# omricarmi/FastHEVC

Measured on AMD Instinct MI355X. Metric: CTU depth decisions/sec at 1080p all-intra + BD-rate delta vs full-RDO HM, higher is better.
Workload: dtype int8 operands / int32 accumulate on v_mfma_i32_32x32x32_i8 (conv2, conv3: 93 % of the MACs); conv1 bf16 operands / f32 accumulate (fixed-point valued); every result exact

## Files before the change

### fasthevc_amd/csrc/k_cnn.hip

```cpp
#include "fhevc_internal.h"
#include <algorithm>
#include <cstdlib>
#include <cstring>

typedef __attribute__((ext_vector_type(8))) short bf16x8;
typedef __attribute__((ext_vector_type(8))) _Float16 f16x8;
typedef __attribute__((ext_vector_type(16))) float f32x16;
typedef __attribute__((ext_vector_type(2))) unsigned short u16x2;

namespace {

constexpr int A1_ROW = 36 * 16;
constexpr int A1_EVEN = 19 * 16;
constexpr int R1_OFF = 0;
constexpr int A3_OFF = R1_OFF;
constexpr int A2_PITCH = 18;
constexpr int A2_PLANE = 18 * 18 * 16 + 192;
constexpr int IN_PITCH = 68;
#ifndef FHEVC_I8_PRIO
#define FHEVC_I8_PRIO 0x0222
#endif
#ifndef FHEVC_F16_PRIO
#define FHEVC_F16_PRIO 0x0123
#endif
// ... 2 lines not shown
#define FHEVC_PRIO_ON(phase)  if (FHEVC_PRIO_OF(phase)) { if (I8) FHEVC_SETPRIO_DYN(1 + prio_slot) else __builtin_amdgcn_s_setprio(FHEVC_PRIO_OF(phase)); }
#define FHEVC_PRIO_OFF(phase) if (FHEVC_PRIO_OF(phase)) __builtin_amdgcn_s_setprio(0);
#ifndef FHEVC_I8_C2_FILL_POOL
#define FHEVC_I8_C2_FILL_POOL 0
#endif
#ifndef FHEVC_I8_C2_FILL_REQUANT
#define FHEVC_I8_C2_FILL_REQUANT 0
#endif
#ifndef FHEVC_I8_C3_FILL
#define FHEVC_I8_C3_FILL 4
#endif
#ifndef FHEVC_I8_C2_FENCE
#define FHEVC_I8_C2_FENCE 0
#endif
#ifndef FHEVC_F16_C2_FILL_POOL
#define FHEVC_F16_C2_FILL_POOL 1
#endif
#ifndef FHEVC_F16_C2_FILL_REQUANT
#define FHEVC_F16_C2_FILL_REQUANT 3
#endif
#ifndef FHEVC_F16_C2_FENCE
#define FHEVC_F16_C2_FENCE 1
#endif
#ifndef FHEVC_I8_C2_SCHED
#define FHEVC_I8_C2_SCHED 1
#endif
#ifndef FHEVC_I8_C3_SCHED
#define FHEVC_I8_C3_SCHED 0
#endif
#ifndef FHEVC_F16_C3_SCHED
#define FHEVC_F16_C3_SCHED 1
#endif
#ifndef FHEVC_CONV1_UNROLL
#define FHEVC_CONV1_UNROLL 2
#endif
#ifndef FHEVC_I8_WG_PER_CU
#define FHEVC_I8_WG_PER_CU 3
#endif
template <bool I8>
struct Lds {
  static constexpr int A1_PLANE = (I8 ? 35 : 34) * A1_ROW;
  static constexpr int A1_PLANES = I8 ? 1 : 2, A2_PLANES = I8 ? 2 : 4;
  static constexpr int R1_BYTES = A1_PLANES * A1_PLANE;
  static constexpr int R2_OFF = R1_OFF + R1_BYTES;
  static constexpr int R2_BYTES = A2_PLANES * A2_PLANE;
  static constexpr int BIAS_OFF = R2_OFF + R2_BYTES;
  static constexpr int LOGIT_OFF = BIAS_OFF + 112 * 4;
  static constexpr int HEADW_OFF = LOGIT_OFF + 64 * 4;
  static constexpr int HADP_OFF = HEADW_OFF + 18432;
  static constexpr int HEADX_OFF = HADP_OFF + 1024;
  static constexpr int LDS_BYTES = HEADX_OFF + 768;
  static constexpr unsigned HALO_FILL = I8 ? 0x80808080u : 0u;
  static_assert(A2_PLANE % 256 == 0, "conv3 reads lane groups of a ds_read_b128 from different planes");
  static_assert(33 * IN_PITCH * 4 + 4 * IN_PITCH * 4 <= R2_BYTES, "input tile (and conv1's one fragment read past it) must fit the A2 region");
  static_assert(HEADW_OFF % 16 == 0, "head weights are read with ds_read_b128");
  static_assert(A3_OFF + 16384 <= R1_OFF + R1_BYTES, "conv3's output must fit R1");
  static_assert(R2_OFF + R2_BYTES <= 65536, "halo offsets are packed into 16 bits");
};
static_assert(2 * Lds<false>::LDS_BYTES <= 160 * 1024, "two workgroups per CU");
static_assert(3 * Lds<true>::LDS_BYTES <= 160 * 1024, "three workgroups per CU");
constexpr int A1_PLANE = Lds<false>::A1_PLANE;

constexpr int HEAD64_OFF = 0, HEAD32_OFF = 2 * 4096, HEAD16_OFF = 4 * 4096;
constexpr int HEADM_OFF = 2 * 4096, HEADM_STEP = 10 * 64, HEADM_BYTES = 16 * HEADM_STEP;

__device__ __forceinline__ float max_with_xor1(float v)
{
  const int o = __builtin_amdgcn_update_dpp(0, __builtin_bit_cast(int, v), 0xB1, 0xF, 0xF, true);
// ... 547 lines not shown
  const int pl = e / 68, k0 = e - pl * 68;
  int y, x;
  if (k0 < 18) { y = 0; x = k0; }
  else if (k0 < 36) { y = 17; x = k0 - 18; }
  else { const int k = k0 - 36; y = 1 + (k >> 1); x = (k & 1) ? 17 : 0; }
  return Lds<I8>::R2_OFF + pl * A2_PLANE + (y * A2_PITCH + x) * 16;
}
template <bool I8>
__device__ __forceinline__ int in_halo_off(int e)
{
  int y, x;
  if (e < 66) { y = 0; x = e; }
  else if (e < 132) { y = 65; x = e - 66; }
  else { const int k = e - 132; y = 1 + (k >> 1); x = (k & 1) ? 65 : 0; }
  return Lds<I8>::R2_OFF + 2 * (2 * ((y >> 1) * IN_PITCH + x) + (y & 1));
}
struct HaloCells { unsigned a1, a2, in; };
template <bool I8>
__device__ __forceinline__ HaloCells halo_cells(int tid)
{
  constexpr int N1 = 132 * Lds<I8>::A1_PLANES, N2 = 68 * Lds<I8>::A2_PLANES;
  HaloCells hc;
  hc.a1 = (unsigned)a1_halo_off<I8>(min(tid, N1 - 1)) | ((unsigned)a1_halo_off<I8>(min(tid + 256, N1 - 1)) << 16);
  hc.a2 = (unsigned)a2_halo_off<I8>(min(tid, N2 - 1)) | ((unsigned)a2_halo_off<I8>(min(tid + 256, N2 - 1)) << 16);
  hc.in = (unsigned)in_halo_off<I8>(tid) | ((unsigned)in_halo_off<I8>(min(tid + 256, 259)) << 16);
  return hc;
}
template <bool I8>
__device__ __forceinline__ void zero_a1_halo(unsigned char* lds, int tid, unsigned cells)
{
  asm volatile("" : "+v"(cells));
  constexpr unsigned Z = Lds<I8>::HALO_FILL;
  *reinterpret_cast<uint4*>(lds + (cells & 0xFFFF)) = make_uint4(Z, Z, Z, Z);
  if (tid < 132 * Lds<I8>::A1_PLANES - 256) *reinterpret_cast<uint4*>(lds + (cells >> 16)) = make_uint4(Z, Z, Z, Z);
}

__device__ __forceinline__ unsigned long long stamp()
{
  unsigned long long t;
  __builtin_amdgcn_sched_barrier(0);
  asm volatile("s_memtime %0\n\ts_waitcnt lgkmcnt(0)" : "=s"(t)::"memory");
  __builtin_amdgcn_sched_barrier(0);
  return t;
}

#define FHEVC_PHASE_IDS                                   \
  int tid = (int)threadIdx.x;                             \
  asm volatile("" : "+v"(tid));                           \
  if (TRIO) tid &= 255;                                   \
  const int lane = tid & 63, wave = tid >> 6;             \
  const int r = lane & 31, h = lane >> 5;                 \
  (void)r; (void)h; (void)wave;

template <bool STAMPS, int HAD, int ARITH, int TRIO = 0>
__global__ __launch_bounds__(TRIO ? 768 : 256, TRIO ? 1 : (ARITH ? FHEVC_I8_WG_PER_CU : 2)) void fhevc_cnn_depth_kernel(FhevcFrames F, FhevcCnnWeights W,
                                                                  uint8_t* __restrict__ d_depth, int32_t* __restrict__ d_had,
                                                                  int32_t* __restrict__ d_logits,
                                                                  uint32_t* __restrict__ d_flags,
                                                                  unsigned long long* __restrict__ d_stamps,
                                                                  uint8_t* __restrict__ d_depth_max, int margin_split, int margin_stop)
{
  extern __shared__ __attribute__((aligned(16))) unsigned char lds_all[];
  const int group = TRIO ? __builtin_amdgcn_readfirstlane((int)(threadIdx.x >> 8)) : 0;
  unsigned char* const lds = lds_all + (TRIO ? group * Lds<ARITH != 0>::LDS_BYTES : 0);
  const int vgrid = TRIO ? 3 * (int)gridDim.x : (int)gridDim.x;
  const int vbidx = TRIO ? group * (int)gridDim.x + (int)blockIdx.x : (int)blockIdx.x;
  __builtin_amdgcn_s_setreg((1 << 11) | 1, 2);
  const int tid = TRIO ? (int)(threadIdx.x & 255) : (int)threadIdx.x;
  const int lane = tid & 63, wave = tid >> 6;
  constexpr bool I8 = ARITH != 0, FASTRQ = ARITH == 2;
  int prio_slot = 0;
  if (I8) {
    const unsigned la = __builtin_amdgcn_s_getreg((31 << 11) | 6);
    const unsigned base = la & 0xFFFu, sz = (la >> 12) & 0x1FFu;
    prio_slot = base >= 2 * sz && sz ? 2 : (base >= sz && sz ? 1 : 0);
    if (TRIO) prio_slot = group;
  }
  (void)prio_slot;
  constexpr bool MFMA_HEADS = I8;
  (void)FASTRQ;
  using L = Lds<I8>;
  const HaloCells hc = halo_cells<I8>(tid);
  const int hb64a = W.bhead[0], hb64b = W.bhead[1] + W.bhead[6 + 0 * 52 + F.qp];
  const int hb32a = W.bhead[2], hb32b = W.bhead[3] + W.bhead[6 + 1 * 52 + F.qp];
  const int hb16a = W.bhead[4], hb16b = W.bhead[5] + W.bhead[6 + 2 * 52 + F.qp];
  const uint4* frag1p = W.frag + FHEVC_FRAG_CONV1 + lane;
  bf16x8 wA1a = __builtin_bit_cast(bf16x8, frag1p[0]);
// ... 106 lines not shown
  if (vblock < total) {
    stage_ctu(lds, L::R2_OFF, pre, F, pos, tid, ld_row, ld_seg, shift_in, hc.in);
    zero_a1_halo<I8>(lds, tid, hc.a1);
    if (HAD == 1) {
      const int hs = F.sample_bytes == 2 ? wave_src_hadamard<2>(pre, lane) : wave_src_hadamard<1>(pre, lane);
      if (lane == 0) logitL[56 + wave] = hs;
    }
  }
  __syncthreads();
  FHEVC_STAMP(0)
  float4 early_b0, early_b1;
  bf16x8 early_bq;
#define FHEVC_CONV1_EARLY_READS                                                                          \
  {                                                                                                      \
    FHEVC_PHASE_IDS                                                                                      \
    early_b0 = *reinterpret_cast<const float4*>(biasL + 8 * h);                                          \
    early_b1 = *reinterpret_cast<const float4*>(biasL + 8 * h + 4);                                      \
    const unsigned char* p = lds + L::R2_OFF + (2 * r + 2 * h) * 4 + wave * (IN_PITCH * 4);              \
    const uint2 lo = *reinterpret_cast<const uint2*>(p);                                                 \
    const uint2 hi = *reinterpret_cast<const uint2*>(p + IN_PITCH * 4);                                  \
    early_bq = __builtin_bit_cast(bf16x8, make_uint4(lo.x, lo.y, hi.x, hi.y));                           \
  }
  FHEVC_CONV1_EARLY_READS
  bf16x8 wH[5];
#define FHEVC_HAD_FRAG_LOADS                                                                                                              \
  if (HAD == 2) {                                                                                                                         \
    unsigned hoff = (unsigned)(threadIdx.x & 63) * 16u + (unsigned)((threadIdx.x >> 6) & 1) * (5u * 64u * 16u);   \
    asm volatile("" : "+v"(hoff));                                                                                                        \
    const unsigned char* hf = reinterpret_cast<const unsigned char*>(W.frag + FHEVC_FRAG_HAD) + hoff;                                     \
    _Pragma("unroll") for (int st = 0; st < 5; ++st) wH[st] = __builtin_bit_cast(bf16x8, *reinterpret_cast<const uint4*>(hf + st * 64 * 16)); \
  }
  FHEVC_HAD_FRAG_LOADS

  if (TRIO) {
    for (int i = 0; i < group; ++i) __syncthreads();
  }
  const int trio_iters = TRIO ? (total + vgrid - 1) / vgrid : 0;
  for (int work = vblock, it = 0; TRIO ? it < trio_iters : work < total; work += vgrid, ++it) {
    if (TRIO && work >= total) {
      __syncthreads(); __syncthreads(); __syncthreads(); __syncthreads();
      continue;
    }
    const int f = pos.f, cy = F.row_begin + pos.ry, cx = pos.cx;
    const CtuPos next = advance(pos, step, band_rows, F.ctus_x);


    {
      FHEVC_PHASE_IDS
      FHEVC_PRIO_ON(0)
      const unsigned char* inb = lds + L::R2_OFF + (2 * r + 2 * h) * 4;
      f32x16 bias1;
      {
        const float4 b0 = early_b0, b1 = early_b1;
        bias1[0] = b0.x; bias1[1] = b0.y; bias1[2] = b0.z; bias1[3] = b0.w;
        bias1[4] = b1.x; bias1[5] = b1.y; bias1[6] = b1.z; bias1[7] = b1.w;
#pragma unroll
        for (int i = 0; i < 8; ++i) bias1[8 + i] = bias1[i];
      }
      auto frag1 = [](const unsigned char* p) {
        const uint2 lo = *reinterpret_cast<const uint2*>(p);
        const uint2 hi = *reinterpret_cast<const uint2*>(p + IN_PITCH * 4);
        return __builtin_bit_cast(bf16x8, make_uint4(lo.x, lo.y, hi.x, hi.y));
      };
      const unsigned char* fp = inb + wave * (IN_PITCH * 4);
      unsigned char* dp = lds + R1_OFF + (I8 ? 8 * h : h * A1_PLANE) + (wave + 1) * A1_ROW + (((r + 1) & 1) ? 0 : A1_EVEN) + ((r + 1) >> 1) * 16;
      bf16x8 bq = early_bq;
      if (HAD == 2) {
        const int mt = wave & 1, nt = wave >> 1;
        const unsigned* hb = reinterpret_cast<const unsigned*>(lds + L::R2_OFF) + (16 * nt + 4 * (r >> 3)) * IN_PITCH + 8 * (r & 7) + 1 + 4 * h;
        f32x16 hacc;
#pragma unroll
        for (int k = 0; k < 16; ++k) hacc[k] = 0.0f;
#pragma unroll
        for (int st = 0; st < 5; ++st) {
          const unsigned* q = hb + st * IN_PITCH;
          const bf16x8 smp = __builtin_bit_cast(bf16x8, make_uint4(q[0], q[1], q[2], q[3]));
          hacc = __builtin_amdgcn_mfma_f32_32x32x16_bf16(wH[st], smp, hacc, 0, 0, 0);
        }
        float t = 0.0f;
#pragma unroll
        for (int k = 0; k < 16; ++k) t += __builtin_fabsf(hacc[k]);
        const u32x2_t sw = __builtin_amdgcn_permlane32_swap(__float_as_uint(t), __float_as_uint(t), false, false);
        t = __uint_as_float(sw.x) + __uint_as_float(sw.y);
        if (h == 0) reinterpret_cast<float*>(lds + L::HADP_OFF)[128 * had_set + 64 * mt + 32 * nt + r] = t;
      }
#pragma unroll FHEVC_CONV1_UNROLL
      for (int i = 0; i < 8; ++i) {
        const f32x16 acc0 = __builtin_amdgcn_mfma_f32_32x32x16_bf16(wA1a, bq, bias1, 0, 0, 0);
        const f32x16 acc1 = __builtin_amdgcn_mfma_f32_32x32x16_bf16(wA1b, bq, bias1, 0, 0, 0);
        fp += 4 * IN_PITCH * 4;
        bq = frag1(fp);
        if (I8) conv1_store_i8(acc0, acc1, dp);
        else conv1_store(acc0, acc1, dp);
        dp += 4 * A1_ROW;
      }
      FHEVC_PRIO_OFF(0)
    }
    __syncthreads();
    FHEVC_STAMP(1)

    if constexpr (I8) {
      FHEVC_PHASE_IDS
      FHEVC_PRIO_ON(1)
      constexpr unsigned Z = L::HALO_FILL;
      unsigned a2cells = hc.a2;
      asm volatile("" : "+v"(a2cells));
      *reinterpret_cast<uint4*>(lds + (a2cells & 0xFFFF)) = make_uint4(Z, Z, Z, Z);
      if (tid < 40) logitL[2 + tid] = tid < 8 ? ((tid & 1) ? hb32b : hb32a) : ((tid & 1) ? hb16b : hb16a);
      const int q = r >> 2;
      const int pr = (q ^ (q >> 1) ^ (q >> 2)) & 1, pc = ((r >> 3) << 2) | (r & 3);
      const unsigned char* a1p = lds + R1_OFF + (2 * pr + h) * A1_ROW + pc * 16;
      unsigned char* a2dst = lds + L::R2_OFF + ((pr + 1) * A2_PITCH + pc + 1) * 16 + 4 * h;
      const int u0 = wave, u1 = wave + 4;
      const unsigned char* h00 = a1p + (4 * u0) * A1_ROW;
      const unsigned char* h10 = a1p + (4 * u1) * A1_ROW;
      const int* b2t = reinterpret_cast<const int*>(biasL) + 16;
      i32x16 t0, t1, a0, a1;
      bf16x8 ring[RINGI];
      const int c2l = conv2_lane_i8(h);
      conv2_half_i8<true, false, 0>(h00, h00 + A1_ROW, c2l, wA2, ring, b2t, h, t0, t1);
      if (FHEVC_I8_C2_SCHED) __builtin_amdgcn_sched_group_barrier(0x100, RINGI + 4, 0);
      if (FHEVC_I8_C2_SCHED) sched_chain12_i8<0>();
      conv2_half_i8<false, false, C2F % RINGI>(h00 + A1_ROW, h10, c2l, wA2, ring, b2t, h, a0, a1);
      pool_h_i8(t0, t1);
// ... 215 lines not shown
        s64b = sdot4(a.x, d1.x, s64b); s64b = sdot4(a.y, d1.y, s64b); s64b = sdot4(a.z, d1.z, s64b); s64b = sdot4(a.w, d1.w, s64b);
      }
      const int r16a = dpp_row_sum(s16a), r16b = dpp_row_sum(s16b);
      const int r32a = dpp_row_sum(s32a), r32b = dpp_row_sum(s32b);
      const int r64a = dpp_row_sum(s64a), r64b = dpp_row_sum(s64b);
      if ((lane & 15) == 0) {
        const int bi = ((q >> 1) * 2 + (blk >> 1)) * 4 + (q & 1) * 2 + (blk & 1);
        *reinterpret_cast<int2*>(logitL + (5 + bi) * 2) = make_int2(r16a + hb16a, r16b + hb16b);
      }
      const int q32a = __builtin_amdgcn_readlane(r32a, 0) + __builtin_amdgcn_readlane(r32a, 16) +
                       __builtin_amdgcn_readlane(r32a, 32) + __builtin_amdgcn_readlane(r32a, 48);
      const int q32b = __builtin_amdgcn_readlane(r32b, 0) + __builtin_amdgcn_readlane(r32b, 16) +
                       __builtin_amdgcn_readlane(r32b, 32) + __builtin_amdgcn_readlane(r32b, 48);
      const int q64a = __builtin_amdgcn_readlane(r64a, 0) + __builtin_amdgcn_readlane(r64a, 16) +
                       __builtin_amdgcn_readlane(r64a, 32) + __builtin_amdgcn_readlane(r64a, 48);
      const int q64b = __builtin_amdgcn_readlane(r64b, 0) + __builtin_amdgcn_readlane(r64b, 16) +
                       __builtin_amdgcn_readlane(r64b, 32) + __builtin_amdgcn_readlane(r64b, 48);
      if (lane == 0) {
        *reinterpret_cast<int2*>(logitL + (1 + q) * 2) = make_int2(q32a + hb32a, q32b + hb32b);
        *reinterpret_cast<int2*>(logitL + 44 + 2 * q) = make_int2(q64a, q64b);
      }
    }
    FHEVC_STAMP(6)
    if (work + vgrid < total) {
      FHEVC_PHASE_IDS
      stage_ctu(lds, L::R2_OFF, pre, F, next, tid, tid >> 2, tid & 3, shift_in, hc.in);
    }
    FHEVC_STAMP(7)
    __syncthreads();
    FHEVC_STAMP(4)
    FHEVC_CONV1_EARLY_READS
    FHEVC_HAD_FRAG_LOADS

    {
      FHEVC_PHASE_IDS
      const int vw = min(64, F.width - cx * 64), vh = min(64, F.height - cy * 64);
      const int ux = tid & 15, uy = tid >> 4;
      const int4 pa = *reinterpret_cast<const int4*>(logitL + 44), pb = *reinterpret_cast<const int4*>(logitL + 48);
      const int2 l64 = make_int2(hb64a + pa.x + pa.z + pb.x + pb.z, hb64b + pa.y + pa.w + pb.y + pb.w);
      const int2 l32 = *reinterpret_cast<const int2*>(logitL + 2 * (1 + (uy >> 3) * 2 + (ux >> 3)));
      const int2 l16 = *reinterpret_cast<const int2*>(logitL + 2 * (5 + (uy >> 2) * 4 + (ux >> 2)));
      const bool e64 = (vw < 64) || (vh < 64);
      bool inside = true, e32 = false, e16 = false;
      if (e64) {
        inside = (ux * 4 < vw) && (uy * 4 < vh);
        e32 = ((ux >> 3) * 32 + 32 > vw) || ((uy >> 3) * 32 + 32 > vh);
        e16 = ((ux >> 2) * 16 + 16 > vw) || ((uy >> 2) * 16 + 16 > vh);
      }
      const int d64 = l64.y - l64.x, d32 = l32.y - l32.x, d16 = l16.y - l16.x;
      const long long o = (long long)(f * band_rows + (cy - F.row_begin)) * F.ctus_x + cx;
      {
        const bool s64 = e64 || d64 > margin_split, s32 = e32 || d32 > margin_split, s16 = e16 || d16 > margin_split;
        const int d = (inside && s64) ? (s32 ? (s16 ? 3 : 2) : 1) : 0;
        d_depth[o * 256 + tid] = (uint8_t)d;
      }
      if (d_depth_max != nullptr) {
        const bool s64 = e64 || d64 > -margin_stop, s32 = e32 || d32 > -margin_stop, s16 = e16 || d16 > -margin_stop;
        const int d = (inside && s64) ? (s32 ? (s16 ? 3 : 2) : 1) : 0;
        d_depth_max[o * 256 + tid] = (uint8_t)d;
      }
      if (d_logits != nullptr && tid < 42) d_logits[o * 42 + tid] = tid == 0 ? l64.x : (tid == 1 ? l64.y : logitL[tid]);
      if (HAD == 1 && tid == 64) {
        const int4 hp = *reinterpret_cast<const int4*>(logitL + 56 + 4 * had_set);
        d_had[o] = hp.x + hp.y + hp.z + hp.w;
      }
      if (HAD == 2 && wave == 1) {
        const float* hp = reinterpret_cast<const float*>(lds + L::HADP_OFF) + 128 * had_set + lane;
        const int sb = (int)(hp[0] + hp[64]);
        int v = dpp_row_sum((sb + 2) >> 2);
        v = __builtin_amdgcn_readlane(v, 0) + __builtin_amdgcn_readlane(v, 16) + __builtin_amdgcn_readlane(v, 32) + __builtin_amdgcn_readlane(v, 48);
        if (lane == 0) d_had[o] = v;
      }
      if (d_flags != nullptr && wave == 0) {
        const int k = lane;
        const int bi = k - 5, qq = k < 5 ? k - 1 : (bi >> 3) * 2 + ((bi >> 1) & 1);
        const int qx = (qq & 1) * 32, qy = (qq >> 1) * 32, bxx = (bi & 3) * 16, byy = (bi >> 2) * 16;
        const int2 a64 = l64;
        const bool n64 = (vw < 64) || (vh < 64) || (a64.y - a64.x > margin_split);
        bool bit = n64;
        if (k >= 1 && k < 21) {
          const int2 a32 = *reinterpret_cast<const int2*>(logitL + 2 * (1 + qq));
          const bool n32 = n64 && (qx < vw) && (qy < vh) && ((qx + 32 > vw) || (qy + 32 > vh) || (a32.y - a32.x > margin_split));
          bit = n32;
          if (k >= 5) {
            const int2 a16 = *reinterpret_cast<const int2*>(logitL + 2 * k);
            bit = n32 && (bxx < vw) && (byy < vh) && ((bxx + 16 > vw) || (byy + 16 > vh) || (a16.y - a16.x > margin_split));
          }
        }
        const unsigned long long m = __ballot(bit && k < 21);
        if (lane == 0) d_flags[o] = (uint32_t)(m & 0x1FFFFFu);
      }
      zero_a1_halo<I8>(lds, tid, hc.a1);
    }
    FHEVC_STAMP(5)
    had_set ^= 1;
    pos = next;
  }
  if (TRIO) {
    for (int i = group; i < 2; ++i) __syncthreads();
  }
  if (STAMPS) {
    unsigned long long treal1;
    const unsigned long long tclk1 = stamp();
    asm volatile("s_memrealtime %0\n\ts_waitcnt lgkmcnt(0)" : "=s"(treal1)::"memory");
    if (tid == 0) {
      for (int k = 0; k < 8; ++k) d_stamps[vbidx * FHEVC_STAMP_SLOTS + k] = tsum[k];
      d_stamps[vbidx * FHEVC_STAMP_SLOTS + 8] = tclk1 - tclk0;
      d_stamps[vbidx * FHEVC_STAMP_SLOTS + 9] = treal1 - treal0;
      d_stamps[vbidx * FHEVC_STAMP_SLOTS + 10] = (unsigned long long)prio_slot;
    }
  }
#undef FHEVC_STAMP
#undef FHEVC_CONV1_EARLY_READS
#undef FHEVC_HAD_FRAG_LOADS
}

__device__ __forceinline__ void depth_map_of_ctu(const FhevcFrames& F, const int* logitL, const int* hads, int tid, int lane, int wave, int f, int cy, int cx,
                                                 int band_rows, int hb64a, int hb64b, int margin_split, int margin_stop, uint8_t* __restrict__ d_depth,
                                                 uint8_t* __restrict__ d_depth_max, int32_t* __restrict__ d_logits, uint32_t* __restrict__ d_flags,
                                                 int32_t* __restrict__ d_had, bool had)
{
  const int vw = min(64, F.width - cx * 64), vh = min(64, F.height - cy * 64);
  const int ux = tid & 15, uy = tid >> 4;
  const int4 pa = *reinterpret_cast<const int4*>(logitL + 44), pb = *reinterpret_cast<const int4*>(logitL + 48);
  const int2 l64 = make_int2(hb64a + pa.x + pa.z + pb.x + pb.z, hb64b + pa.y + pa.w + pb.y + pb.w);
  const int2 l32 = *reinterpret_cast<const int2*>(logitL + 2 * (1 + (uy >> 3) * 2 + (ux >> 3)));
  const int2 l16 = *reinterpret_cast<const int2*>(logitL + 2 * (5 + (uy >> 2) * 4 + (ux >> 2)));
  const bool e64 = (vw < 64) || (vh < 64);
  bool inside = true, e32 = false, e16 = false;
  if (e64) {
    inside = (ux * 4 < vw) && (uy * 4 < vh);
    e32 = ((ux >> 3) * 32 + 32 > vw) || ((uy >> 3) * 32 + 32 > vh);
    e16 = ((ux >> 2) * 16 + 16 > vw) || ((uy >> 2) * 16 + 16 > vh);
  }
  const int d64 = l64.y - l64.x, d32 = l32.y - l32.x, d16 = l16.y - l16.x;
  const long long o = (long long)(f * band_rows + (cy - F.row_begin)) * F.ctus_x + cx;
  {
    const bool s64 = e64 || d64 > margin_split, s32 = e32 || d32 > margin_split, s16 = e16 || d16 > margin_split;
    const int d = (inside && s64) ? (s32 ? (s16 ? 3 : 2) : 1) : 0;
    d_depth[o * 256 + tid] = (uint8_t)d;
  }
  if (d_depth_max != nullptr) {
    const bool s64 = e64 || d64 > -margin_stop, s32 = e32 || d32 > -margin_stop, s16 = e16 || d16 > -margin_stop;
    const int d = (inside && s64) ? (s32 ? (s16 ? 3 : 2) : 1) : 0;
    d_depth_max[o * 256 + tid] = (uint8_t)d;
  }
// ... 34 lines not shown
  const int tid = threadIdx.x, uy = tid & 15, sub = tid >> 4;
  for (long long c = (long long)blockIdx.x * 16 + sub; c < total; c += (long long)gridDim.x * 16) {
    const int rem = (int)(c % per_frame), cy = rem / F.ctus_x, cx = rem - cy * F.ctus_x;
    const int vw = min(64, F.width - cx * 64), vh = min(64, F.height - cy * 64);
    const uint32_t w = flags[c];
    uint32_t out[4] = { 0, 0, 0, 0 };
    if (uy * 4 < vh && (w & 1u)) {
#pragma unroll
      for (int j = 0; j < 4; ++j) {
        const int q = (uy >> 3) * 2 + (j >> 1), bi = (uy >> 2) * 4 + j;
        const uint32_t d = ((w >> (1 + q)) & 1u) ? (((w >> (5 + bi)) & 1u) ? 3u : 2u) : 1u;
        const int nvalid = min(4, max(0, (vw >> 2) - 4 * j));
        out[j] = (d * 0x01010101u) & (nvalid >= 4 ? 0xFFFFFFFFu : ((1u << (8 * nvalid)) - 1u));
      }
    }
    *reinterpret_cast<uint4*>(depth + c * 256 + uy * 16) = make_uint4(out[0], out[1], out[2], out[3]);
  }
}

}

hipError_t fhevc_launch_expand_flags(const FhevcFrames& fr, const uint32_t* d_flags, uint8_t* d_depth, hipStream_t stream)
{
  const long long total = (long long)fr.ctus_x * fr.ctus_y * fr.num_frames;
  if (total <= 0) return hipSuccess;
  const long long groups = (total + 15) / 16;
  const int grid = (int)(groups < 8192 ? groups : 8192);
  hipLaunchKernelGGL(fhevc_expand_flags_kernel, dim3(grid), dim3(256), 0, stream, fr, d_flags, d_depth);
  return hipGetLastError();
}

hipError_t fhevc_cnn_prepare_device()
{
  hipError_t e = hipFuncSetAttribute(reinterpret_cast<const void*>(&fhevc_cnn_depth_kernel<false, 0, 0>), hipFuncAttributeMaxDynamicSharedMemorySize, Lds<false>::LDS_BYTES);
  if (e == hipSuccess) e = hipFuncSetAttribute(reinterpret_cast<const void*>(&fhevc_cnn_depth_kernel<false, 1, 0>), hipFuncAttributeMaxDynamicSharedMemorySize, Lds<false>::LDS_BYTES);
  if (e == hipSuccess) e = hipFuncSetAttribute(reinterpret_cast<const void*>(&fhevc_cnn_depth_kernel<false, 2, 0>), hipFuncAttributeMaxDynamicSharedMemorySize, Lds<false>::LDS_BYTES);
  if (e == hipSuccess) e = hipFuncSetAttribute(reinterpret_cast<const void*>(&fhevc_cnn_family_kernel<32, 64, 128>), hipFuncAttributeMaxDynamicSharedMemorySize, LdsFam<32, 64, 128>::LDS_BYTES);
  if (e == hipSuccess) e = hipFuncSetAttribute(reinterpret_cast<const void*>(&fhevc_cnn_family_kernel<16, 32, 64>), hipFuncAttributeMaxDynamicSharedMemorySize, LdsFam<16, 32, 64>::LDS_BYTES);
#define FHEVC_LAYER_LDS(KCV) \
  if (e == hipSuccess) e = hipFuncSetAttribute(reinterpret_cast<const void*>(&fhevc_layer_conv_kernel<KCV, false, true>), hipFuncAttributeMaxDynamicSharedMemorySize, 80 * 1024); \
  if (e == hipSuccess) e = hipFuncSetAttribute(reinterpret_cast<const void*>(&fhevc_layer_conv_kernel<KCV, true, true>), hipFuncAttributeMaxDynamicSharedMemorySize, 80 * 1024);
  FHEVC_LAYER_LDS(1) FHEVC_LAYER_LDS(2) FHEVC_LAYER_LDS(3) FHEVC_LAYER_LDS(4)
#undef FHEVC_LAYER_LDS
#define FHEVC_LAYER_FUSE(KCV) \
  if (e == hipSuccess) e = hipFuncSetAttribute(reinterpret_cast<const void*>(&fhevc_layer_conv_kernel<KCV, false, true, true>), hipFuncAttributeMaxDynamicSharedMemorySize, 80 * 1024); \
  if (e == hipSuccess) e = hipFuncSetAttribute(reinterpret_cast<const void*>(&fhevc_layer_conv_kernel<KCV, true, true, true>), hipFuncAttributeMaxDynamicSharedMemorySize, 80 * 1024);
  FHEVC_LAYER_FUSE(1) FHEVC_LAYER_FUSE(2)
#undef FHEVC_LAYER_FUSE
  if (e == hipSuccess) e = hipFuncSetAttribute(reinterpret_cast<const void*>(&fhevc_cnn_d2_kernel<1, 2, 3, false>), hipFuncAttributeMaxDynamicSharedMemorySize, LdsD2<1, 2, 3>::LDS_BYTES);
  if (e == hipSuccess) e = hipFuncSetAttribute(reinterpret_cast<const void*>(&fhevc_cnn_d2_kernel<1, 2, 3, true>), hipFuncAttributeMaxDynamicSharedMemorySize, LdsD2<1, 2, 3>::LDS_BYTES);
  if (e == hipSuccess) e = hipFuncSetAttribute(reinterpret_cast<const void*>(&fhevc_cnn_depth_kernel<false, 0, 2, 1>), hipFuncAttributeMaxDynamicSharedMemorySize, 3 * Lds<true>::LDS_BYTES);
  if (e == hipSuccess) e = hipFuncSetAttribute(reinterpret_cast<const void*>(&fhevc_cnn_depth_kernel<false, 1, 2, 1>), hipFuncAttributeMaxDynamicSharedMemorySize, 3 * Lds<true>::LDS_BYTES);
  if (e == hipSuccess) e = hipFuncSetAttribute(reinterpret_cast<const void*>(&fhevc_cnn_depth_kernel<true, 1, 2, 1>), hipFuncAttributeMaxDynamicSharedMemorySize, 3 * Lds<true>::LDS_BYTES);
  return e;
}

bool fhevc_cnn_can_fuse_hadamard(const FhevcFrames& fr)
{
  const size_t sb = (size_t)fr.sample_bytes;
  return fr.bit_depth <= 10 && (fr.width % 16) == 0 && (fr.height % 8) == 0 && (reinterpret_cast<uintptr_t>(fr.luma) % 16) == 0 &&
         ((size_t)fr.stride * sb) % 16 == 0 && ((size_t)fr.frame_stride * sb) % 16 == 0;
}

namespace {
template <bool STAMPS, int HAD, int ARITH>
void launch_depth_kernel(int grid, hipStream_t stream, const FhevcFrames& fr, const FhevcCnnWeights& w, uint8_t* d_depth, int32_t* d_had, int32_t* d_logits,
                         uint32_t* d_flags, unsigned long long* d_stamps, uint8_t* d_depth_max, int margin_split, int margin_stop)
{
  hipLaunchKernelGGL((fhevc_cnn_depth_kernel<STAMPS, HAD, ARITH>), dim3(grid), dim3(256), Lds<ARITH != 0>::LDS_BYTES, stream, fr, w, d_depth, d_had, d_logits,
                     d_flags, d_stamps, d_depth_max, margin_split, margin_stop);
}
int cnn_arith(const FhevcCnnWeights& w) { return !w.i8 ? 0 : (w.requant_mode[1] == 1 && w.requant_mode[2] == 2) ? 2 : 1; }
}

FhevcKnobs fhevc_read_knobs()
{
  FhevcKnobs k;
  auto digit = [](const char* e) { return (e && e[0] >= '1' && e[0] <= '4') ? e[0] - '0' : 0; };
  k.wg_per_cu = digit(std::getenv("FHEVC_CNN_WG_PER_CU"));
  k.debug_wg_per_cu = digit(std::getenv("FHEVC_DEBUG_WG_PER_CU"));
  if (const char* rq = std::getenv("FHEVC_CNN_REQUANT")) k.requant_general = std::strcmp(rq, "general") == 0;
  k.family_layers = std::getenv("FHEVC_FAMILY_LAYERS") != nullptr;
  if (const char* fd = std::getenv("FHEVC_FUSED_D2")) k.fused_d2 = fd[0] != '0';
  k.layers_no_fuse = std::getenv("FHEVC_LAYERS_NO_FUSE") != nullptr;
  k.layers_no_dbuf = std::getenv("FHEVC_LAYERS_NO_DBUF") != nullptr;
  if (const char* kb = std::getenv("FHEVC_LAYERS_LDS_KB")) k.layers_lds_limit = (size_t)std::min(80, std::max(8, std::atoi(kb))) * 1024;
  if (const char* lg = std::getenv("FHEVC_LAYERS_GRID")) k.layers_grid = std::atoi(lg);
  if (const char* tr = std::getenv("FHEVC_CNN_TRIO")) k.trio = tr[0] != '0';
  if (const char* rq = std::getenv("FHEVC_D2_REQUANT")) k.d2_requant_general = std::strcmp(rq, "general") == 0;
  return k;
}

static int cnn_wg_per_cu(const FhevcCnnWeights& w, const FhevcKnobs& knobs)
{
  if (knobs.wg_per_cu) return knobs.wg_per_cu;
  return w.i8 ? FHEVC_I8_WG_PER_CU : 2;
}

hipError_t fhevc_launch_cnn(const FhevcFrames& fr, const FhevcCnnWeights& w, uint8_t* d_depth, int32_t* d_had, int32_t* d_logits,
                            uint32_t* d_flags, uint8_t* d_depth_max, int margin_split, int margin_stop, int num_cus, const FhevcKnobs& knobs, hipStream_t stream)
{
  const long long total = (long long)(fr.row_end - fr.row_begin) * fr.ctus_x * fr.num_frames;
  if (total <= 0) return hipSuccess;
  int grid = cnn_wg_per_cu(w, knobs) * num_cus;
  if (total < grid) grid = (int)total;
#define FHEVC_LAUNCH(HAD, ARITH) launch_depth_kernel<false, HAD, ARITH>(grid, stream, fr, w, d_depth, d_had, d_logits, d_flags, nullptr, d_depth_max, margin_split, margin_stop)
  const int had = d_had == nullptr ? 0 : (fr.bit_depth == 8 && !w.had_valu) ? 2 : 1;
  if (knobs.trio && !knobs.wg_per_cu && cnn_arith(w) == 2 && had != 2) {
    const int tgrid = (int)std::min<long long>(num_cus, (total + 2) / 3);
#define FHEVC_LAUNCH_TRIO(HAD) hipLaunchKernelGGL((fhevc_cnn_depth_kernel<false, HAD, 2, 1>), dim3(tgrid), dim3(768), 3 * Lds<true>::LDS_BYTES, stream, fr, w, d_depth, d_had, \
                                                  d_logits, d_flags, nullptr, d_depth_max, margin_split, margin_stop)
    if (had) FHEVC_LAUNCH_TRIO(1); else FHEVC_LAUNCH_TRIO(0);
#undef FHEVC_LAUNCH_TRIO
    return hipGetLastError();
  }
#define FHEVC_LAUNCH_HAD(ARITH) do { if (had == 2) FHEVC_LAUNCH(2, ARITH); else if (had == 1) FHEVC_LAUNCH(1, ARITH); else FHEVC_LAUNCH(0, ARITH); } while (0)
  switch (cnn_arith(w)) {
    case 2: FHEVC_LAUNCH_HAD(2); break;
    case 1: FHEVC_LAUNCH_HAD(1); break;
    default: FHEVC_LAUNCH_HAD(0); break;
  }
#undef FHEVC_LAUNCH_HAD
#undef FHEVC_LAUNCH
  return hipGetLastError();
}

hipError_t fhevc_launch_cnn_stamped(const FhevcFrames& fr, const FhevcCnnWeights& w, uint8_t* d_depth, int32_t* d_had, int num_cus, const FhevcKnobs& knobs,
                                    unsigned long long* d_stamps, int* grid_out, hipStream_t stream)
{
  const long long total = (long long)(fr.row_end - fr.row_begin) * fr.ctus_x * fr.num_frames;
  int grid = (knobs.debug_wg_per_cu ? knobs.debug_wg_per_cu : cnn_wg_per_cu(w, knobs)) * num_cus;
  if (total < grid) grid = (int)total;
  *grid_out = grid;
  if (total <= 0) return hipSuccess;
  const int arith = cnn_arith(w);
  if (arith == 0) {
    hipError_t e = hipFuncSetAttribute(reinterpret_cast<const void*>(&fhevc_cnn_depth_kernel<true, 0, 0>), hipFuncAttributeMaxDynamicSharedMemorySize, Lds<false>::LDS_BYTES);
    if (e != hipSuccess) return e;
    launch_depth_kernel<true, 0, 0>(grid, stream, fr, w, d_depth, nullptr, nullptr, nullptr, d_stamps, nullptr, 0, 0);
  } else if (arith == 1) launch_depth_kernel<true, 0, 1>(grid, stream, fr, w, d_depth, nullptr, nullptr, nullptr, d_stamps, nullptr, 0, 0);
  else if (d_had && knobs.trio && !knobs.debug_wg_per_cu && !knobs.wg_per_cu) {
    const int tgrid = (int)std::min<long long>(num_cus, (total + 2) / 3);
    *grid_out = 3 * tgrid;
    hipLaunchKernelGGL((fhevc_cnn_depth_kernel<true, 1, 2, 1>), dim3(tgrid), dim3(768), 3 * Lds<true>::LDS_BYTES, stream, fr, w, d_depth, d_had, nullptr, nullptr, d_stamps, nullptr, 0, 0);
  } else if (d_had) launch_depth_kernel<true, 1, 2>(grid, stream, fr, w, d_depth, d_had, nullptr, nullptr, d_stamps, nullptr, 0, 0);
  else launch_depth_kernel<true, 0, 2>(grid, stream, fr, w, d_depth, nullptr, nullptr, nullptr, d_stamps, nullptr, 0, 0);
  return hipGetLastError();
}

bool fhevc_cnn_family_supported(int c1, int c2, int c3) { return (c1 == 32 && c2 == 64 && c3 == 128) || (c1 == 16 && c2 == 32 && c3 == 64); }

hipError_t fhevc_launch_cnn_family(const FhevcFrames& fr, const FhevcFamilyWeights& w, uint8_t* d_depth, int32_t* d_logits, uint32_t* d_flags,
                                   uint8_t* d_depth_max, int margin_split, int margin_stop, int num_cus, hipStream_t stream)
{
  const long long total = (long long)(fr.row_end - fr.row_begin) * fr.ctus_x * fr.num_frames;
  if (total <= 0) return hipSuccess;
  int grid = 2 * num_cus;
  if (total < grid) grid = (int)total;
  if (w.c[0] == 32 && w.c[1] == 64 && w.c[2] == 128)
    hipLaunchKernelGGL((fhevc_cnn_family_kernel<32, 64, 128>), dim3(grid), dim3(256), (LdsFam<32, 64, 128>::LDS_BYTES), stream, fr, w, d_depth, d_logits, d_flags, d_depth_max, margin_split, margin_stop);
  else if (w.c[0] == 16 && w.c[1] == 32 && w.c[2] == 64)
    hipLaunchKernelGGL((fhevc_cnn_family_kernel<16, 32, 64>), dim3(grid), dim3(256), (LdsFam<16, 32, 64>::LDS_BYTES), stream, fr, w, d_depth, d_logits, d_flags, d_depth_max, margin_split, margin_stop);
  else return hipErrorInvalidValue;
  return hipGetLastError();
}

bool fhevc_cnn_d2_supported(const FhevcLayersWeights& w)
{
  static const int cp[6] = { 32, 32, 64, 64, 96, 96 }, pool[6] = { 0, 1, 0, 1, 0, 0 }, hh[6] = { 64, 64, 32, 32, 16, 16 };
  if (w.num_layers != 6 || w.c3_pad != 96) return false;
  for (int i = 0; i < 6; ++i)
    if (w.l[i].cout_pad != cp[i] || (w.l[i].pool != 0) != (pool[i] != 0) || w.l[i].H != hh[i] || w.l[i].kc != (i == 0 ? 0 : cp[i - 1] / 32)) return false;
  return true;
}

hipError_t fhevc_launch_cnn_d2(const FhevcFrames& fr, const FhevcLayersWeights& w, uint8_t* d_depth, int32_t* d_logits, uint32_t* d_flags,
                               uint8_t* d_depth_max, int margin_split, int margin_stop, int num_cus, hipStream_t stream)
// ... 79 lines not shown
```

Measured before the change: 89.28 million.

## Defer depth-map tail into next CTU's conv1 loop and add plain-output variant

Moves the per-CTU depth decision and output stores (depth, had, flags, logits) out of the end of each iteration. The logits are read into registers at iteration end, and the tail then runs inside the first unrolled unit of the next CTU's conv1 loop, with a final flush after the loop. The aim is to hide the tail's global stores and scalar work behind conv1 MFMAs. Conv1 unroll is raised to 8, branchy edge checks are made branch-free, and stores go through buffer resources so a dead tail becomes a no-op. A PLAIN template variant drops the optional outputs when they are null, at the cost of more register pressure and more kernel instantiations.

After: 89.13 million. No clear change (-0.2%).

```diff
diff --git a/fasthevc_amd/csrc/k_cnn.hip b/fasthevc_amd/csrc/k_cnn.hip
--- a/fasthevc_amd/csrc/k_cnn.hip
+++ b/fasthevc_amd/csrc/k_cnn.hip
@@ -58,8 +58,9 @@
 #define FHEVC_F16_C3_SCHED 1
 #endif
 #ifndef FHEVC_CONV1_UNROLL
-#define FHEVC_CONV1_UNROLL 2
+#define FHEVC_CONV1_UNROLL 8
 #endif
+static_assert(FHEVC_CONV1_UNROLL == 8, "the depth-map tail sits in the first of conv1's unrolled units");
 #ifndef FHEVC_I8_WG_PER_CU
 #define FHEVC_I8_WG_PER_CU 3
 #endif
@@ -673,7 +674,9 @@
   asm volatile("" : "+v"(cells));
   constexpr unsigned Z = Lds<I8>::HALO_FILL;
   *reinterpret_cast<uint4*>(lds + (cells & 0xFFFF)) = make_uint4(Z, Z, Z, Z);
-  if (tid < 132 * Lds<I8>::A1_PLANES - 256) *reinterpret_cast<uint4*>(lds + (cells >> 16)) = make_uint4(Z, Z, Z, Z);
+  if constexpr (132 * Lds<I8>::A1_PLANES > 256) {
+    if (tid < 132 * Lds<I8>::A1_PLANES - 256) *reinterpret_cast<uint4*>(lds + (cells >> 16)) = make_uint4(Z, Z, Z, Z);
+  }
 }
 
 __device__ __forceinline__ unsigned long long stamp()
@@ -693,7 +696,7 @@
   const int r = lane & 31, h = lane >> 5;                 \
   (void)r; (void)h; (void)wave;
 
-template <bool STAMPS, int HAD, int ARITH, int TRIO = 0>
+template <bool STAMPS, int HAD, int ARITH, int TRIO = 0, bool PLAIN = false>
 __global__ __launch_bounds__(TRIO ? 768 : 256, TRIO ? 1 : (ARITH ? FHEVC_I8_WG_PER_CU : 2)) void fhevc_cnn_depth_kernel(FhevcFrames F, FhevcCnnWeights W,
                                                                   uint8_t* __restrict__ d_depth, int32_t* __restrict__ d_had,
                                                                   int32_t* __restrict__ d_logits,
@@ -866,6 +869,84 @@
   }
   FHEVC_HAD_FRAG_LOADS
 
+  struct TailIn { int4 pa, pb; int2 l32, l16; int4 hp; };
+  TailIn tin = { make_int4(0, 0, 0, 0), make_int4(0, 0, 0, 0), make_int2(0, 0), make_int2(0, 0), make_int4(0, 0, 0, 0) };
+  int tail_o = -1, tail_dims = 0;
+#define FHEVC_TAIL_READS                                                                                   \
+  {                                                                                                        \
+    FHEVC_PHASE_IDS                                                                                        \
+    const int ux = tid & 15, uy = tid >> 4;                                                                \
+    tin.pa = *reinterpret_cast<const int4*>(logitL + 44);                                                  \
+    tin.pb = *reinterpret_cast<const int4*>(logitL + 48);                                                  \
+    tin.l32 = *reinterpret_cast<const int2*>(logitL + 2 * (1 + (uy >> 3) * 2 + (ux >> 3)));               \
+    tin.l16 = *reinterpret_cast<const int2*>(logitL + 2 * (5 + (uy >> 2) * 4 + (ux >> 2)));               \
+    if (HAD == 1) tin.hp = *reinterpret_cast<const int4*>(logitL + 56 + 4 * had_set);                      \
+  }
+  constexpr int OOB = (int)0x80000000u;
+  auto depth_tail = [&]() __attribute__((always_inline)) {
+    FHEVC_PHASE_IDS
+    const int o = tail_o, vw = tail_dims & 0xFF, vh = tail_dims >> 8;
+    const bool live = o >= 0;
+    const size_t ob = (size_t)(live ? o : 0);
+    const int ux = tid & 15, uy = tid >> 4;
+    const int4 pa = tin.pa, pb = tin.pb;
+    const int2 l64 = make_int2(hb64a + pa.x + pa.z + pb.x + pb.z, hb64b + pa.y + pa.w + pb.y + pb.w);
+    const int2 l32 = tin.l32, l16 = tin.l16;
+    const bool e64 = (vw < 64) || (vh < 64);
+    const bool inside = (ux * 4 < vw) && (uy * 4 < vh);
+    const bool e32 = ((ux >> 3) * 32 + 32 > vw) || ((uy >> 3) * 32 + 32 > vh);
+    const bool e16 = ((ux >> 2) * 16 + 16 > vw) || ((uy >> 2) * 16 + 16 > vh);
+    const int d64 = l64.y - l64.x, d32 = l32.y - l32.x, d16 = l16.y - l16.x;
+    {
+      const bool s64 = e64 || d64 > margin_split, s32 = e32 || d32 > margin_split, s16 = e16 || d16 > margin_split;
+      const int d = (inside && s64) ? (s32 ? (s16 ? 3 : 2) : 1) : 0;
+      const __amdgpu_buffer_rsrc_t rd = __builtin_amdgcn_make_buffer_rsrc(d_depth + ob * 256, 0, live ? 256 : 0, 0x00020000);
+      __builtin_amdgcn_raw_buffer_store_b8((unsigned char)d, rd, tid, 0, 0);
+    }
+    if constexpr (!PLAIN) {
+      if (live) {
+        if (d_depth_max != nullptr) {
+          const bool s64 = e64 || d64 > -margin_stop, s32 = e32 || d32 > -margin_stop, s16 = e16 || d16 > -margin_stop;
+          const int d = (inside && s64) ? (s32 ? (s16 ? 3 : 2) : 1) : 0;
+          d_depth_max[ob * 256 + tid] = (uint8_t)d;
+        }
+        if (d_logits != nullptr && tid < 42) d_logits[ob * 42 + tid] = tid == 0 ? l64.x : (tid == 1 ? l64.y : logitL[tid]);
+        if (d_flags != nullptr && wave == 0) {
+          const int k = lane;
+          const int bi = k - 5, qq = k < 5 ? k - 1 : (bi >> 3) * 2 + ((bi >> 1) & 1);
+          const int qx = (qq & 1) * 32, qy = (qq >> 1) * 32, bxx = (bi & 3) * 16, byy = (bi >> 2) * 16;
+          const int2 a64 = l64;
+          const bool n64 = (vw < 64) || (vh < 64) || (a64.y - a64.x > margin_split);
+          bool bit = n64;
+          if (k >= 1 && k < 21) {
+            const int2 a32 = *reinterpret_cast<const int2*>(logitL + 2 * (1 + qq));
+            const bool n32 = n64 && (qx < vw) && (qy < vh) && ((qx + 32 > vw) || (qy + 32 > vh) || (a32.y - a32.x > margin_split));
+            bit = n32;
+            if (k >= 5) {
+              const int2 a16 = *reinterpret_cast<const int2*>(logitL + 2 * k);
+              bit = n32 && (bxx < vw) && (byy < vh) && ((bxx + 16 > vw) || (byy + 16 > vh) || (a16.y - a16.x > margin_split));
+            }
+          }
+          const unsigned long long m = __ballot(bit && k < 21);
+          if (lane == 0) d_flags[ob] = (uint32_t)(m & 0x1FFFFFu);
+        }
+      }
+    }
+    if (HAD == 1) {
+      const __amdgpu_buffer_rsrc_t rh = __builtin_amdgcn_make_buffer_rsrc(d_had + ob, 0, live ? 4 : 0, 0x00020000);
+      __builtin_amdgcn_raw_buffer_store_b32(tin.hp.x + tin.hp.y + tin.hp.z + tin.hp.w, rh, tid == 64 ? 0 : OOB, 0, 0);
+    }
+    if (HAD == 2 && wave == 1) {
+      const float* hp = reinterpret_cast<const float*>(lds + L::HADP_OFF) + 128 * (had_set ^ 1) + lane;
+      const int sb = (int)(hp[0] + hp[64]);
+      int v = dpp_row_sum((sb + 2) >> 2);
+      v = __builtin_amdgcn_readlane(v, 0) + __builtin_amdgcn_readlane(v, 16) + __builtin_amdgcn_readlane(v, 32) + __builtin_amdgcn_readlane(v, 48);
+      const __amdgpu_buffer_rsrc_t rh = __builtin_amdgcn_make_buffer_rsrc(d_had + ob, 0, live ? 4 : 0, 0x00020000);
+      __builtin_amdgcn_raw_buffer_store_b32(v, rh, lane == 0 ? 0 : OOB, 0, 0);
+    }
+    zero_a1_halo<I8>(lds, tid, hc.a1);
+  };
+
   if (TRIO) {
     for (int i = 0; i < group; ++i) __syncthreads();
   }
@@ -924,6 +1005,11 @@
         const f32x16 acc1 = __builtin_amdgcn_mfma_f32_32x32x16_bf16(wA1b, bq, bias1, 0, 0, 0);
         fp += 4 * IN_PITCH * 4;
         bq = frag1(fp);
+        if (i == 0) {
+          FHEVC_STAMP(1)
+          depth_tail();
+          FHEVC_STAMP(5)
+        }
         if (I8) conv1_store_i8(acc0, acc1, dp);
         else conv1_store(acc0, acc1, dp);
         dp += 4 * A1_ROW;
@@ -1205,70 +1291,14 @@
     FHEVC_CONV1_EARLY_READS
     FHEVC_HAD_FRAG_LOADS
 
-    {
-      FHEVC_PHASE_IDS
-      const int vw = min(64, F.width - cx * 64), vh = min(64, F.height - cy * 64);
-      const int ux = tid & 15, uy = tid >> 4;
-      const int4 pa = *reinterpret_cast<const int4*>(logitL + 44), pb = *reinterpret_cast<const int4*>(logitL + 48);
-      const int2 l64 = make_int2(hb64a + pa.x + pa.z + pb.x + pb.z, hb64b + pa.y + pa.w + pb.y + pb.w);
-      const int2 l32 = *reinterpret_cast<const int2*>(logitL + 2 * (1 + (uy >> 3) * 2 + (ux >> 3)));
-      const int2 l16 = *reinterpret_cast<const int2*>(logitL + 2 * (5 + (uy >> 2) * 4 + (ux >> 2)));
-      const bool e64 = (vw < 64) || (vh < 64);
-      bool inside = true, e32 = false, e16 = false;
-      if (e64) {
-        inside = (ux * 4 < vw) && (uy * 4 < vh);
-        e32 = ((ux >> 3) * 32 + 32 > vw) || ((uy >> 3) * 32 + 32 > vh);
-        e16 = ((ux >> 2) * 16 + 16 > vw) || ((uy >> 2) * 16 + 16 > vh);
-      }
-      const int d64 = l64.y - l64.x, d32 = l32.y - l32.x, d16 = l16.y - l16.x;
-      const long long o = (long long)(f * band_rows + (cy - F.row_begin)) * F.ctus_x + cx;
-      {
-        const bool s64 = e64 || d64 > margin_split, s32 = e32 || d32 > margin_split, s16 = e16 || d16 > margin_split;
-        const int d = (inside && s64) ? (s32 ? (s16 ? 3 : 2) : 1) : 0;
-        d_depth[o * 256 + tid] = (uint8_t)d;
-      }
-      if (d_depth_max != nullptr) {
-        const bool s64 = e64 || d64 > -margin_stop, s32 = e32 || d32 > -margin_stop, s16 = e16 || d16 > -margin_stop;
-        const int d = (inside && s64) ? (s32 ? (s16 ? 3 : 2) : 1) : 0;
-        d_depth_max[o * 256 + tid] = (uint8_t)d;
-      }
-      if (d_logits != nullptr && tid < 42) d_logits[o * 42 + tid] = tid == 0 ? l64.x : (tid == 1 ? l64.y : logitL[tid]);
-      if (HAD == 1 && tid == 64) {
-        const int4 hp = *reinterpret_cast<const int4*>(logitL + 56 + 4 * had_set);
-        d_had[o] = hp.x + hp.y + hp.z + hp.w;
-      }
-      if (HAD == 2 && wave == 1) {
-        const float* hp = reinterpret_cast<const float*>(lds + L::HADP_OFF) + 128 * had_set + lane;
-        const int sb = (int)(hp[0] + hp[64]);
-        int v = dpp_row_sum((sb + 2) >> 2);
-        v = __builtin_amdgcn_readlane(v, 0) + __builtin_amdgcn_readlane(v, 16) + __builtin_amdgcn_readlane(v, 32) + __builtin_amdgcn_readlane(v, 48);
-        if (lane == 0) d_had[o] = v;
-      }
-      if (d_flags != nullptr && wave == 0) {
-        const int k = lane;
-        const int bi = k - 5, qq = k < 5 ? k - 1 : (bi >> 3) * 2 + ((bi >> 1) & 1);
-        const int qx = (qq & 1) * 32, qy = (qq >> 1) * 32, bxx = (bi & 3) * 16, byy = (bi >> 2) * 16;
-        const int2 a64 = l64;
-        const bool n64 = (vw < 64) || (vh < 64) || (a64.y - a64.x > margin_split);
-        bool bit = n64;
-        if (k >= 1 && k < 21) {
-          const int2 a32 = *reinterpret_cast<const int2*>(logitL + 2 * (1 + qq));
-          const bool n32 = n64 && (qx < vw) && (qy < vh) && ((qx + 32 > vw) || (qy + 32 > vh) || (a32.y - a32.x > margin_split));
-          bit = n32;
-          if (k >= 5) {
-            const int2 a16 = *reinterpret_cast<const int2*>(logitL + 2 * k);
-            bit = n32 && (bxx < vw) && (byy < vh) && ((bxx + 16 > vw) || (byy + 16 > vh) || (a16.y - a16.x > margin_split));
-          }
-        }
-        const unsigned long long m = __ballot(bit && k < 21);
-        if (lane == 0) d_flags[o] = (uint32_t)(m & 0x1FFFFFu);
-      }
-      zero_a1_halo<I8>(lds, tid, hc.a1);
-    }
-    FHEVC_STAMP(5)
+    FHEVC_TAIL_READS
+    tail_o = (f * band_rows + pos.ry) * F.ctus_x + cx;
+    tail_dims = min(64, F.width - cx * 64) | (min(64, F.height - cy * 64) << 8);
     had_set ^= 1;
     pos = next;
   }
+  depth_tail();
+  FHEVC_STAMP(5)
   if (TRIO) {
     for (int i = group; i < 2; ++i) __syncthreads();
   }
@@ -1285,6 +1315,7 @@
   }
 #undef FHEVC_STAMP
 #undef FHEVC_CONV1_EARLY_READS
+#undef FHEVC_TAIL_READS
 #undef FHEVC_HAD_FRAG_LOADS
 }
 
@@ -1385,9 +1416,11 @@
 
 hipError_t fhevc_cnn_prepare_device()
 {
-  hipError_t e = hipFuncSetAttribute(reinterpret_cast<const void*>(&fhevc_cnn_depth_kernel<false, 0, 0>), hipFuncAttributeMaxDynamicSharedMemorySize, Lds<false>::LDS_BYTES);
-  if (e == hipSuccess) e = hipFuncSetAttribute(reinterpret_cast<const void*>(&fhevc_cnn_depth_kernel<false, 1, 0>), hipFuncAttributeMaxDynamicSharedMemorySize, Lds<false>::LDS_BYTES);
-  if (e == hipSuccess) e = hipFuncSetAttribute(reinterpret_cast<const void*>(&fhevc_cnn_depth_kernel<false, 2, 0>), hipFuncAttributeMaxDynamicSharedMemorySize, Lds<false>::LDS_BYTES);
+  hipError_t e = hipSuccess;
+#define FHEVC_DEPTH_LDS(HAD, ARITH, TRIO, BYTES) \
+  if (e == hipSuccess) e = hipFuncSetAttribute(reinterpret_cast<const void*>(&fhevc_cnn_depth_kernel<false, HAD, ARITH, TRIO, false>), hipFuncAttributeMaxDynamicSharedMemorySize, BYTES); \
+  if (e == hipSuccess) e = hipFuncSetAttribute(reinterpret_cast<const void*>(&fhevc_cnn_depth_kernel<false, HAD, ARITH, TRIO, true>), hipFuncAttributeMaxDynamicSharedMemorySize, BYTES);
+  FHEVC_DEPTH_LDS(0, 0, 0, Lds<false>::LDS_BYTES) FHEVC_DEPTH_LDS(1, 0, 0, Lds<false>::LDS_BYTES) FHEVC_DEPTH_LDS(2, 0, 0, Lds<false>::LDS_BYTES)
   if (e == hipSuccess) e = hipFuncSetAttribute(reinterpret_cast<const void*>(&fhevc_cnn_family_kernel<32, 64, 128>), hipFuncAttributeMaxDynamicSharedMemorySize, LdsFam<32, 64, 128>::LDS_BYTES);
   if (e == hipSuccess) e = hipFuncSetAttribute(reinterpret_cast<const void*>(&fhevc_cnn_family_kernel<16, 32, 64>), hipFuncAttributeMaxDynamicSharedMemorySize, LdsFam<16, 32, 64>::LDS_BYTES);
 #define FHEVC_LAYER_LDS(KCV) \
@@ -1402,9 +1435,9 @@
 #undef FHEVC_LAYER_FUSE
   if (e == hipSuccess) e = hipFuncSetAttribute(reinterpret_cast<const void*>(&fhevc_cnn_d2_kernel<1, 2, 3, false>), hipFuncAttributeMaxDynamicSharedMemorySize, LdsD2<1, 2, 3>::LDS_BYTES);
   if (e == hipSuccess) e = hipFuncSetAttribute(reinterpret_cast<const void*>(&fhevc_cnn_d2_kernel<1, 2, 3, true>), hipFuncAttributeMaxDynamicSharedMemorySize, LdsD2<1, 2, 3>::LDS_BYTES);
-  if (e == hipSuccess) e = hipFuncSetAttribute(reinterpret_cast<const void*>(&fhevc_cnn_depth_kernel<false, 0, 2, 1>), hipFuncAttributeMaxDynamicSharedMemorySize, 3 * Lds<true>::LDS_BYTES);
-  if (e == hipSuccess) e = hipFuncSetAttribute(reinterpret_cast<const void*>(&fhevc_cnn_depth_kernel<false, 1, 2, 1>), hipFuncAttributeMaxDynamicSharedMemorySize, 3 * Lds<true>::LDS_BYTES);
-  if (e == hipSuccess) e = hipFuncSetAttribute(reinterpret_cast<const void*>(&fhevc_cnn_depth_kernel<true, 1, 2, 1>), hipFuncAttributeMaxDynamicSharedMemorySize, 3 * Lds<true>::LDS_BYTES);
+  FHEVC_DEPTH_LDS(0, 2, 1, 3 * Lds<true>::LDS_BYTES) FHEVC_DEPTH_LDS(1, 2, 1, 3 * Lds<true>::LDS_BYTES)
+#undef FHEVC_DEPTH_LDS
+  if (e == hipSuccess) e = hipFuncSetAttribute(reinterpret_cast<const void*>(&fhevc_cnn_depth_kernel<true, 1, 2, 1, true>), hipFuncAttributeMaxDynamicSharedMemorySize, 3 * Lds<true>::LDS_BYTES);
   return e;
 }
 
@@ -1416,11 +1449,11 @@
 }
 
 namespace {
-template <bool STAMPS, int HAD, int ARITH>
+template <bool STAMPS, int HAD, int ARITH, bool PLAIN = STAMPS>
 void launch_depth_kernel(int grid, hipStream_t stream, const FhevcFrames& fr, const FhevcCnnWeights& w, uint8_t* d_depth, int32_t* d_had, int32_t* d_logits,
                          uint32_t* d_flags, unsigned long long* d_stamps, uint8_t* d_depth_max, int margin_split, int margin_stop)
 {
-  hipLaunchKernelGGL((fhevc_cnn_depth_kernel<STAMPS, HAD, ARITH>), dim3(grid), dim3(256), Lds<ARITH != 0>::LDS_BYTES, stream, fr, w, d_depth, d_had, d_logits,
+  hipLaunchKernelGGL((fhevc_cnn_depth_kernel<STAMPS, HAD, ARITH, 0, PLAIN>), dim3(grid), dim3(256), Lds<ARITH != 0>::LDS_BYTES, stream, fr, w, d_depth, d_had, d_logits,
                      d_flags, d_stamps, d_depth_max, margin_split, margin_stop);
 }
 int cnn_arith(const FhevcCnnWeights& w) { return !w.i8 ? 0 : (w.requant_mode[1] == 1 && w.requant_mode[2] == 2) ? 2 : 1; }
@@ -1457,13 +1490,16 @@
   if (total <= 0) return hipSuccess;
   int grid = cnn_wg_per_cu(w, knobs) * num_cus;
   if (total < grid) grid = (int)total;
-#define FHEVC_LAUNCH(HAD, ARITH) launch_depth_kernel<false, HAD, ARITH>(grid, stream, fr, w, d_depth, d_had, d_logits, d_flags, nullptr, d_depth_max, margin_split, margin_stop)
+  const bool plain = d_depth_max == nullptr && d_logits == nullptr && d_flags == nullptr;
+#define FHEVC_LAUNCH_AS(HAD, ARITH, PLAIN) launch_depth_kernel<false, HAD, ARITH, PLAIN>(grid, stream, fr, w, d_depth, d_had, d_logits, d_flags, nullptr, d_depth_max, margin_split, margin_stop)
+#define FHEVC_LAUNCH(HAD, ARITH) do { if (plain) FHEVC_LAUNCH_AS(HAD, ARITH, true); else FHEVC_LAUNCH_AS(HAD, ARITH, false); } while (0)
   const int had = d_had == nullptr ? 0 : (fr.bit_depth == 8 && !w.had_valu) ? 2 : 1;
   if (knobs.trio && !knobs.wg_per_cu && cnn_arith(w) == 2 && had != 2) {
     const int tgrid = (int)std::min<long long>(num_cus, (total + 2) / 3);
-#define FHEVC_LAUNCH_TRIO(HAD) hipLaunchKernelGGL((fhevc_cnn_depth_kernel<false, HAD, 2, 1>), dim3(tgrid), dim3(768), 3 * Lds<true>::LDS_BYTES, stream, fr, w, d_depth, d_had, \
-                                                  d_logits, d_flags, nullptr, d_depth_max, margin_split, margin_stop)
-    if (had) FHEVC_LAUNCH_TRIO(1); else FHEVC_LAUNCH_TRIO(0);
+#define FHEVC_LAUNCH_TRIO(HAD, PLAIN) hipLaunchKernelGGL((fhevc_cnn_depth_kernel<false, HAD, 2, 1, PLAIN>), dim3(tgrid), dim3(768), 3 * Lds<true>::LDS_BYTES, stream, fr, w, d_depth, d_had, \
+                                                         d_logits, d_flags, nullptr, d_depth_max, margin_split, margin_stop)
+    if (had) { if (plain) FHEVC_LAUNCH_TRIO(1, true); else FHEVC_LAUNCH_TRIO(1, false); }
+    else { if (plain) FHEVC_LAUNCH_TRIO(0, true); else FHEVC_LAUNCH_TRIO(0, false); }
 #undef FHEVC_LAUNCH_TRIO
     return hipGetLastError();
   }
@@ -1475,6 +1511,7 @@
   }
 #undef FHEVC_LAUNCH_HAD
 #undef FHEVC_LAUNCH
+#undef FHEVC_LAUNCH_AS
   return hipGetLastError();
 }
 
@@ -1488,14 +1525,14 @@
   if (total <= 0) return hipSuccess;
   const int arith = cnn_arith(w);
   if (arith == 0) {
-    hipError_t e = hipFuncSetAttribute(reinterpret_cast<const void*>(&fhevc_cnn_depth_kernel<true, 0, 0>), hipFuncAttributeMaxDynamicSharedMemorySize, Lds<false>::LDS_BYTES);
+    hipError_t e = hipFuncSetAttribute(reinterpret_cast<const void*>(&fhevc_cnn_depth_kernel<true, 0, 0, 0, true>), hipFuncAttributeMaxDynamicSharedMemorySize, Lds<false>::LDS_BYTES);
     if (e != hipSuccess) return e;
     launch_depth_kernel<true, 0, 0>(grid, stream, fr, w, d_depth, nullptr, nullptr, nullptr, d_stamps, nullptr, 0, 0);
   } else if (arith == 1) launch_depth_kernel<true, 0, 1>(grid, stream, fr, w, d_depth, nullptr, nullptr, nullptr, d_stamps, nullptr, 0, 0);
   else if (d_had && knobs.trio && !knobs.debug_wg_per_cu && !knobs.wg_per_cu) {
     const int tgrid = (int)std::min<long long>(num_cus, (total + 2) / 3);
     *grid_out = 3 * tgrid;
-    hipLaunchKernelGGL((fhevc_cnn_depth_kernel<true, 1, 2, 1>), dim3(tgrid), dim3(768), 3 * Lds<true>::LDS_BYTES, stream, fr, w, d_depth, d_had, nullptr, nullptr, d_stamps, nullptr, 0, 0);
+    hipLaunchKernelGGL((fhevc_cnn_depth_kernel<true, 1, 2, 1, true>), dim3(tgrid), dim3(768), 3 * Lds<true>::LDS_BYTES, stream, fr, w, d_depth, d_had, nullptr, nullptr, d_stamps, nullptr, 0, 0);
   } else if (d_had) launch_depth_kernel<true, 1, 2>(grid, stream, fr, w, d_depth, d_had, nullptr, nullptr, d_stamps, nullptr, 0, 0);
   else launch_depth_kernel<true, 0, 2>(grid, stream, fr, w, d_depth, nullptr, nullptr, nullptr, d_stamps, nullptr, 0, 0);
   return hipGetLastError();
```
